# rendeirolab/stainx

Measured on AMD Instinct MI355X. Metric: megapixels/sec Macenko transform, 64x3x512x512 fp32; max-abs vs torch CPU, higher is better.
Workload: dtype f32; 1 GPU; Macenko reference-mode transform, 64x3x512x512 fp32 per GPU (BASELINE configs[1]); tiles_per_gpu=64, height=512, width=512, input_batches_rotated=2, parallelism=tiles sharded over 1 GPU(s), no collective

## Files before the change

stainx_amd/csrc/macenko.hip:

```cpp
#include "common.hpp"

#include <algorithm>
#include <atomic>
#include <type_traits>
#include <cstdlib>

namespace sx {
namespace macenko {

constexpr int kSample = 4096;
constexpr int kMinCap = 8192;
constexpr int kChunk = 16384;
template <typename T> struct PackOf { static constexpr int n = 16 / (int)sizeof(T); };
constexpr int kSlots = 4;
constexpr int kMoments = 20;
constexpr int kPartial = 10;
constexpr int kShortList = 512;
constexpr int kGroupThreads = 1024;
constexpr int kKeys = kSample / kGroupThreads;
constexpr int kPrefetchHist = 8;
constexpr int kPrefetchCand = 8;
static_assert(kKeys * kGroupThreads == kSample && kPrefetchCand * kGroupThreads <= kMinCap, "per-tile stage geometry");

constexpr float kBeta = 0.15f;
// ... 258 lines not shown
        __syncthreads();
    }
};
template <typename F> struct Coded {
    uint8_t v;
    __device__ __forceinline__ operator uint32_t() const { return v; }
};
template <typename T> struct Sem { using type = T; };
template <typename F> struct Sem<Coded<F>> { using type = F; };
template <typename F> __device__ __forceinline__ float code_value(int k) {
    return Elem<F>::load(Elem<F>::store(div255_of_level((float)k)));
}
template <typename F> struct LevelTables<Coded<F>> {
    float od[256], l2[256];
    __device__ __forceinline__ void fill() {
        for (int t = threadIdx.x; t < 256; t += blockDim.x) {
            const float v = code_value<F>(t);
            od[t] = optical_density<F>(v);
            l2[t] = log2_level<F>(v);
        }
        __syncthreads();
    }
};
template <typename F, int kCodeCopies> struct CodeTable {
    static constexpr int copies = kCodeCopies;
    uint2 e[256 * kCodeCopies];
    __device__ __forceinline__ void fill() {
        for (int t = threadIdx.x; t < 256; t += blockDim.x) {
            const float v = code_value<F>(t);
            const uint2 entry = make_uint2(__float_as_uint(v), __float_as_uint(optical_density<F>(v)));
#pragma unroll
            for (int c = 0; c < kCodeCopies; ++c) e[t * kCodeCopies + c] = entry;
        }
        __syncthreads();
    }
};
template <typename T, int V, bool kInter> struct Codable { static constexpr bool value = std::is_same<T, float>::value && V == 4 && !kInter; };

template <typename T> __device__ __forceinline__ float od_of(float v, const LevelTables<T>& tb) {
    if constexpr (sizeof(T) == 1) return tb.od[__float_as_uint(v)]; else return optical_density<T>(v);
}
template <typename T> __device__ __forceinline__ float l2_of(float v, const LevelTables<T>& tb) {
    if constexpr (sizeof(T) == 1) return tb.l2[__float_as_uint(v)]; else return log2_level<T>(v);
}

__device__ __forceinline__ bool od_selected(const float od[3], bool use_all) {
    return use_all || (fminf(od[0], fminf(od[1], od[2])) >= kBeta);
}

__device__ __forceinline__ float diamond_angle(float t1, float t0) {
    const float den = fmaxf(fabsf(t0) + fabsf(t1), 1e-30f);
    const float r = t1 * __builtin_amdgcn_rcpf(den);
    return t0 >= 0.0f ? r : (t1 >= 0.0f ? 2.0f - r : -2.0f - r);
// ... 147 lines not shown
        }
        return out;
    }
};
__device__ __forceinline__ bool in_mask(uint32_t mask_bits, int i) { return ((mask_bits >> i) & 1u) != 0u; }
__device__ __forceinline__ uint32_t* mask_count_words(const Workspace& ws, int64_t item) { return ws.block_hist + (size_t)item * 512; }
__device__ __forceinline__ float sample_out_of_mask() { return __uint_as_float(0x7FC00000u); }
__device__ __forceinline__ bool sample_in_mask(const float od[3]) { return od[0] == od[0]; }

template <typename T> __device__ __forceinline__ float input_level(float held) {
    if constexpr (sizeof(T) == 1) return (float)__float_as_uint(held); else return held * 255.0f;
}

template <int W>
__device__ __forceinline__ void store_codes(const Geometry& g, const Workspace& ws, int64_t tile, int64_t p, const uint32_t (&word)[3][W]) {
    static_assert(W == 1 || W == 2, "four or eight codes per plane");
#pragma unroll
    for (int c = 0; c < 3; ++c) {
        uint8_t* dst = ws.codes + ((size_t)tile * 3 + c) * g.pixels + p;
        if constexpr (W == 1) *reinterpret_cast<uint32_t*>(dst) = word[c][0]; else *reinterpret_cast<uint2*>(dst) = make_uint2(word[c][0], word[c][1]);
    }
}
template <typename T, int V, bool kInter, class Table>
__device__ __forceinline__ void code_quad(const PixelPacks<T, V, kInter>& u, int i0, const LevelTables<T>& tb, const Table& ct, const Geometry& g, const Workspace& ws, int64_t tile, float (&od_quad)[4][3], uint32_t (&word)[3][V / 4]) {
    static_assert((V == 4 || V == 8) && !kInter, "a pack's codes are one or two 32-bit words of a plane");
    constexpr int kCodeCopies = Table::copies;
    uint32_t differ = 0u;
    const int copy = (int)(threadIdx.x % kCodeCopies);
#pragma unroll
    for (int c = 0; c < 3; ++c) {
        uint32_t w = 0u;
#pragma unroll
        for (int ii = 0; ii < 4; ++ii) {
            const float x = u.value(c, i0 + ii);
            const uint32_t k = __float_as_uint(fmaf(x, 255.0f, 8388608.0f)) & 0xFFu;
            const uint2 entry = ct.e[k * kCodeCopies + copy];
            differ |= entry.x ^ __float_as_uint(x);
            od_quad[ii][c] = __uint_as_float(entry.y);
            w |= k << (8 * ii);
        }
        word[c][i0 / 4] = w;
    }
    if (__builtin_expect(__builtin_amdgcn_ballot_w64(differ != 0u) != 0ull, 0)) {
#pragma unroll
        for (int ii = 0; ii < 4; ++ii)
#pragma unroll
            for (int c = 0; c < 3; ++c) {
                float x = u.value(c, i0 + ii);
                asm volatile("" : "+v"(x));
                od_quad[ii][c] = od_of<T>(x, tb);
            }
        if (differ != 0u) put(&ws.code_bad[tile], g.code_epoch);
    }
}


template <typename O, int V, bool kInter>
__device__ __forceinline__ void store_pixels(O* __restrict__ dst, int64_t pixels, int64_t p, const O (&res)[3][V]) {
    if constexpr (kInter) {
        O flat[3][V];
#pragma unroll
        for (int i = 0; i < V; ++i)
#pragma unroll
            for (int c = 0; c < 3; ++c) flat[(3 * i + c) / V][(3 * i + c) % V] = res[c][i];
#pragma unroll
        for (int k = 0; k < 3; ++k) store_pack_stream<O, V>(dst + 3 * p + k * V, flat[k]);
    } else {
#pragma unroll
        for (int c = 0; c < 3; ++c) store_pack_stream<O, V>(dst + c * pixels + p, res[c]);
    }
}

template <typename O, int V>
__device__ __forceinline__ void store_pixels_staged(O* __restrict__ dst, int64_t p, const O (&res)[3][V], uint4* __restrict__ stage) {
    static_assert(sizeof(O) * V == 16, "16-byte packs");
// ... 4338 lines not shown
```

stainx_amd/csrc/macenko_twopass.hpp:

```cpp
#pragma once

namespace sx {
namespace macenko {

constexpr int kPriorSweeps = 4;
constexpr int kPriorUnitsMax = kGroupThreads / 4 * kPriorSweeps;
constexpr int kQueue2 = 512;
constexpr float kSpecSigmasConc = 5.0f, kSpecThresholdScale = 1.0f;
constexpr float kSpecSigmas = 5.0f;
constexpr float kSpecEffFar = 2.0f, kSpecEffNear = 1.0f;
__device__ __forceinline__ float spec_eff(const Geometry& g) { return g.prior_step_q16 >= (8u << 16) ? g.spec_eff_far : g.spec_eff_near; }
constexpr float kSpecKw = 0.10f, kSpecKx = 1.3e-3f;
constexpr float kSpecRot = 0.30f;
constexpr uint32_t kSpecSlow = 1u, kSpecHazard = 2u;
constexpr int kMaxSegments = 256;

constexpr int kRowBelowA = 0, kRowAboveA = 1, kRowBelowB = 2, kRowAboveB = 3, kRowConc = 4, kRowW = 8;
struct alignas(128) PriorRecord {
    float a0[3], a1[3], an[3];
    float rows[16][4];
    float kw, kx;
    float cmax[4];
    int32_t mode;
    int32_t min_first;
    uint32_t open;
};

struct alignas(64) FusedTile {
    uint32_t a_done;
    uint32_t s_done;
    uint32_t ncand[kSlots];
    uint32_t pad[10];
};
constexpr int kXcds = 8;
struct alignas(64) FusedQueue {
    uint32_t ticket;
    uint32_t pad[15];
};
struct FusedSched {
    FusedQueue queue[kXcds];
};
static_assert(sizeof(FusedTile) == kFusedTileBytes && sizeof(FusedSched) <= kFusedSchedBytes, "workspace layout");


typedef unsigned int sx_u4 __attribute__((ext_vector_type(4)));
__device__ __forceinline__ uint32_t ld_agent(const uint32_t* p) { return __hip_atomic_load(p, __ATOMIC_RELAXED, __HIP_MEMORY_SCOPE_AGENT); }
__device__ __forceinline__ int32_t ld_agent(const int32_t* p) { return __hip_atomic_load(p, __ATOMIC_RELAXED, __HIP_MEMORY_SCOPE_AGENT); }
__device__ __forceinline__ float ld_agent(const float* p) { return __uint_as_float(__hip_atomic_load(reinterpret_cast<const uint32_t*>(p), __ATOMIC_RELAXED, __HIP_MEMORY_SCOPE_AGENT)); }
// ... 2 lines not shown
}
__device__ __forceinline__ void st_agent(uint32_t* p, uint32_t v) { __hip_atomic_store(p, v, __ATOMIC_RELAXED, __HIP_MEMORY_SCOPE_AGENT); }
__device__ __forceinline__ void st_agent(float* p, float v) { __hip_atomic_store(reinterpret_cast<uint32_t*>(p), __float_as_uint(v), __ATOMIC_RELAXED, __HIP_MEMORY_SCOPE_AGENT); }
__device__ __forceinline__ void st_agent(double* p, double v) {
    __hip_atomic_store(reinterpret_cast<unsigned long long*>(p), (unsigned long long)__double_as_longlong(v), __ATOMIC_RELAXED, __HIP_MEMORY_SCOPE_AGENT);
}
__device__ __forceinline__ void drain_stores() { asm volatile("s_waitcnt vmcnt(0)" ::: "memory"); }

constexpr int kPriorBins = 2048;
constexpr int kPriorAnglePlane = 4;
constexpr float kOpenExponent = 30.0f;
constexpr float kOpenNear = 16.0f;
struct alignas(16) PriorScratch {
    double red[kGroupThreads / kWave][kPartial];
    double mom[kMoments];
    uint32_t hist[5][kPriorBins];
    uint32_t od16[kPriorSweeps][6][kGroupThreads];
    uint32_t n_kept, n_all, hazard, r_max;
    float frame[9];
    float bdir[4][2];
    float bkey[4], blevel[4];
    uint32_t cmax[4];
    uint32_t open;
};

__device__ __forceinline__ uint32_t prior_pick_bin(const uint32_t* hist, uint32_t rank) {
    constexpr int kPer = kPriorBins / kWave;
    static_assert(kPer <= kWave, "second level: one bin per lane");
    const int lane = (int)lane_id();
    uint32_t mine = 0;
#pragma unroll 8
    for (int i = 0; i < kPer; ++i) mine += hist[kPer * lane + i];
    const uint32_t incl = wave_scan_u32(mine);
    const uint64_t over = __ballot(incl > rank);
    const int owner = over ? (__ffsll((long long)over) - 1) : (kWave - 1);
    const uint32_t r = rank - (uint32_t)__builtin_amdgcn_readlane((int)(incl - mine), owner);
    const uint32_t h = lane < kPer ? hist[kPer * owner + lane] : 0u;
    const uint32_t incl2 = wave_scan_u32(h);
    const uint64_t over2 = __ballot(lane < kPer && incl2 > r);
    const int sub = over2 ? (__ffsll((long long)over2) - 1) : (kPer - 1);
    return (uint32_t)(kPer * owner + sub);
}

__device__ __forceinline__ float wave_total_f32(float x) {
    auto step = [](float v, auto mover) { return v + __uint_as_float(mover(__float_as_uint(v))); };
    x = step(x, [](uint32_t b) { return dpp_move<0x111, 0xF>(0u, b); });
// ... 19 lines not shown
#pragma unroll
        for (int i = 0; i < 4; ++i) {
            float v[3][1];
            load_pixels<T, 1, kInter>(img, g.pixels, p + i, v);
#pragma unroll
            for (int c = 0; c < 3; ++c) u[c][i] = v[c][0];
        }
    }
    return have;
}
template <typename T>
__device__ __forceinline__ void prior_densities(const float (&u)[3][4], float (&od)[4][3]) {
#pragma unroll
    for (int i = 0; i < 4; ++i)
#pragma unroll
        for (int c = 0; c < 3; ++c) od[i][c] = optical_density<T>(u[c][i]);
}

template <typename T, bool kVec, bool kInter>
__global__ __launch_bounds__(kGroupThreads) void prior_kernel(const T* __restrict__ images, Geometry g, Workspace ws) {
    __shared__ PriorScratch sh;
    const int tile = blockIdx.x, tid = threadIdx.x, wave = tid / kWave;
    const uint32_t lane = lane_id();
    GroupState& st = ws.state[tile];
    PriorRecord* pr = &ws.prior[tile];
    const T* img = images + (int64_t)tile * 3 * g.pixels;
    SX_STAMP(st, 0);
    if (tid < kSlots) {
        put(&st.ncand[tid], 0u);
        put(&st.below[tid], 0u);
        put(&st.ncand_seen[tid], 0u);
        put(&st.over_count[tid], 0u);
    }
    if (tid < 2) put(&st.phi_pub[tid], 0ull);
    if ((g.fused || g.dense) && tid < (int)(sizeof(FusedTile) / 4)) put(reinterpret_cast<uint32_t*>(&ws.ftile[tile]) + tid, 0u);
    if (g.fused && tile == 0 && tid >= 32 && tid < 32 + kXcds) put(&ws.fsched->queue[tid - 32].ticket, 0u);
    if (tid == 0) {
        put(&st.fell_back, 0u);
        put(&st.spec, 0u);
        sh.n_kept = sh.n_all = sh.hazard = sh.open = sh.r_max = 0;
        sh.cmax[0] = sh.cmax[1] = sh.cmax[2] = sh.cmax[3] = 0;
    }
    for (int i = tid; i < 5 * kPriorBins; i += kGroupThreads) (&sh.hist[0][0])[i] = 0;

    {
        float m[kPartial];
#pragma unroll
        for (int k = 0; k < kPartial; ++k) m[k] = 0.0f;
        float raw[kPriorSweeps][3][4];
        bool have_quad[kPriorSweeps];
#pragma unroll
        for (int s = 0; s < kPriorSweeps; ++s) have_quad[s] = prior_fetch<T, kVec, kInter>(img, g, s, raw[s]);
#pragma unroll
        for (int s = 0; s < kPriorSweeps; ++s) {
            float od[4][3];
            prior_densities<T>(raw[s], od);
            const bool have = have_quad[s];
#pragma unroll
            for (int q = 0; q < 6; ++q) {
                const int e = 2 * q;
                typedef __fp16 fp16x2 __attribute__((ext_vector_type(2)));
                const fp16x2 h = __builtin_amdgcn_cvt_pkrtz(od[e / 3][e % 3], od[(e + 1) / 3][(e + 1) % 3]);
                sh.od16[s][q][tid] = __builtin_bit_cast(uint32_t, h);
            }
#pragma unroll
            for (int i = 0; i < 4; ++i) {
                const float* o = od[i];
                const float keep = (have && od_selected(o, false)) ? 1.0f : 0.0f;
                const float k0 = keep * o[0], k1 = keep * o[1], k2 = keep * o[2];
                m[0] += keep;
                m[1] += k0;
                m[2] += k1;
                m[3] += k2;
                m[4] = fmaf(k0, o[0], m[4]);
                m[5] = fmaf(k0, o[1], m[5]);
                m[6] = fmaf(k0, o[2], m[6]);
                m[7] = fmaf(k1, o[1], m[7]);
                m[8] = fmaf(k1, o[2], m[8]);
                m[9] = fmaf(k2, o[2], m[9]);
            }
        }
        SX_STAMP(st, 1);
#pragma unroll
        for (int k = 0; k < kPartial; ++k) {
            const float s = wave_total_f32(m[k]);
            if (lane == kWave - 1) sh.red[wave][k] = (double)s;
        }
    }
    __syncthreads();
    if (tid < kMoments) {
        double s = 0.0;
        if (tid < kPartial)
            for (int w = 0; w < kGroupThreads / kWave; ++w) s += sh.red[w][tid];
        sh.mom[tid] = s;
    }
    __syncthreads();
    const int m_kept = (int)sh.mom[0];
    SX_STAMP(st, 2);
    if (tid < 2 && m_kept >= 3) {
        double cov[9];
        float vecs[6];
        bool use_all;
        unsigned long long n_sel;
        plane_from_moments<true>(sh.mom, false, cov, vecs, use_all, n_sel);
        if (tid == 0) {
            const double x0 = vecs[0], y0 = vecs[2], z0 = vecs[4], x1 = vecs[1], y1 = vecs[3], z1 = vecs[5];
            double nx = y0 * z1 - z0 * y1, ny = z0 * x1 - x0 * z1, nz = x0 * y1 - y0 * x1;
            const double n2 = nx * nx + ny * ny + nz * nz;
            const double inv = n2 > 0.0 ? 1.0 / sqrt(n2) : 0.0;
            sh.frame[0] = vecs[0]; sh.frame[1] = vecs[2]; sh.frame[2] = vecs[4];
            sh.frame[3] = vecs[1]; sh.frame[4] = vecs[3]; sh.frame[5] = vecs[5];
            sh.frame[6] = (float)(nx * inv); sh.frame[7] = (float)(ny * inv); sh.frame[8] = (float)(nz * inv);
        }
    }
    __syncthreads();
    auto give_up = [&]() {
        if (tid == 0) {
// ... 261 lines not shown
    for (int s = 0; s < kSlots; ++s) at0[s] = (uint32_t)__builtin_amdgcn_readlane((int)base, s);
    const auto rsrc = __builtin_amdgcn_make_buffer_rsrc(rec_tile, 0, (int)(kSlots * cap * 16u), 0x00020000);
    for (uint32_t i0 = 0; i0 < n; i0 += kWave) {
        const uint32_t i = i0 + lane;
        sx_u4 rec = {0u, 0u, 0u, 0u};
        uint32_t flags = 0;
        if (i < n) {
            rec[0] = queue[0][i];
            rec[1] = queue[1][i];
            rec[2] = queue[2][i];
            flags = queue[3][i];
        }
#pragma unroll
        for (int s = 0; s < kSlots; ++s) {
            const bool has = ((flags >> s) & 1u) != 0;
            const uint64_t mask = __builtin_amdgcn_ballot_w64(has);
            const uint32_t at = at0[s] + rank_in_mask(mask);
            if (has && at < cap) __builtin_amdgcn_raw_buffer_store_b128(rec, rsrc, (int)(((uint32_t)s * cap + at) * 16u), 0, 16);
            at0[s] += (uint32_t)__popcll(mask);
        }
    }
}

template <typename T, int V, int TPB, bool kInter, bool kFused = false, bool kEmit = false>
__device__ __forceinline__ void pass_a_item(const T* __restrict__ images, const Geometry& g, const Workspace& ws, int64_t tile, int chunk_id, int64_t item, PassAScratch<TPB>* sh, const LevelTables<T>& tb,
                                            const CodeTable<T, 2>* __restrict__ ct = nullptr) {
    const int64_t p_begin = (int64_t)chunk_id * g.chunk;
    const int64_t p_end = min(p_begin + (int64_t)g.chunk, g.pixels);
    const T* img = images + tile * 3 * g.pixels;
    GroupState& st = ws.state[tile];
    const PriorRecord* __restrict__ pr = &ws.prior[tile];
    const int wave = __builtin_amdgcn_readfirstlane((int)(threadIdx.x / kWave));
    const bool speculate = get(&pr->mode) == 0;
    typedef _Float16 half8 __attribute__((ext_vector_type(8)));
    typedef float float16v __attribute__((ext_vector_type(16)));
    half8 test_rows;
    {
        const uint32_t l = lane_id(), r = l & 31u, h = l >> 5, row_half = (r >> 2) & 1u, test = (r & 3u) + 4u * (r >> 3);
        const float4 coef = *reinterpret_cast<const float4*>(&pr->rows[test][0]);
        const bool mine = h == row_half;
        test_rows[0] = (_Float16)(mine ? coef.x : 0.0f);
        test_rows[1] = (_Float16)(mine ? coef.y : 0.0f);
        test_rows[2] = (_Float16)(mine ? coef.z : 0.0f);
        test_rows[3] = (_Float16)(mine ? coef.w : 0.0f);
        test_rows[4] = test_rows[5] = test_rows[6] = test_rows[7] = (_Float16)0.0f;
    }
    const float kw = get(&pr->kw), kx = get(&pr->kx);
    if (threadIdx.x < 2) sh->below[threadIdx.x] = 0;

    constexpr int kShortRun = 32 / V > 0 ? 32 / V : 1;
    double acc[kPartial];
#pragma unroll
    for (int k = 0; k < kPartial; ++k) acc[k] = 0.0;
    float m[kPartial];
#pragma unroll
    for (int k = 0; k < kPartial; ++k) m[k] = 0.0f;

    uint32_t (*queue)[kQueue2] = sh->queue[wave];
    uint32_t n_q = 0, have[kSlots] = {0u, 0u, 0u, 0u}, below_a = 0, below_b = 0;
    float* cand_tile = ws.cand_od + (size_t)tile * kSlots * 3 * g.cap2;
    const uint32_t seg = (uint32_t)chunk_id * (TPB / kWave) + (uint32_t)wave, seg_base = seg * g.seg_cap;
    auto flush = [&]() {
        if constexpr (kFused)
            write_records_fused(queue, n_q, ws.cand_rec + (size_t)tile * kSlots * g.fused_cap, g.fused_cap, ws.ftile[tile].ncand);
        else
            write_records(queue, n_q, have, cand_tile, g, seg_base, st.over_count);
        n_q = 0;
    };

    const int64_t mine = (int64_t)threadIdx.x * V;
    PixelPacks<T, V, kInter> next;
    next.clear();
    if (p_begin + mine < p_end) next.load(img, g.pixels, p_begin + mine);
    __syncthreads();

    int in_run = 0;
    auto sweep = [&](auto with_tests) {
        constexpr bool kTests = decltype(with_tests)::value;
        constexpr int G = 1;
        for (int64_t base_p = p_begin; base_p < p_end; base_p += (int64_t)TPB * V) {
            const bool live = base_p + mine < p_end;
            const PixelPacks<T, V, kInter> u = next;
            const int64_t p_next = base_p + (int64_t)TPB * V + mine;
            if (p_next < p_end) next.load(img, g.pixels, p_next);
            uint64_t live_mask = __builtin_amdgcn_ballot_w64(live);
            asm volatile("" : "+s"(live_mask));
            float od_quad[4][3];
            if constexpr (kEmit) {
                static_assert(!kEmit || V == 4, "one quad per pack");
                if (live) {
                    uint32_t word[3][1];
                    code_quad(u, 0, tb, *ct, g, ws, tile, od_quad, word);
                    store_codes<1>(g, ws, tile, base_p + mine, word);
                }
            }
#pragma unroll
            for (int i0 = 0; i0 < V; i0 += G) {
                float od[G][3];
                uint64_t valid[G];
                float16v forms[G];
#pragma unroll
                for (int gi = 0; gi < G; ++gi) {
#pragma unroll
                    for (int c = 0; c < 3; ++c) {
                        if constexpr (kEmit) od[gi][c] = od_quad[(i0 + gi) % 4][c]; else od[gi][c] = od_of<T>(u.value(c, i0 + gi), tb);
                    }
                    const bool sel = od_selected(od[gi], false);
                    valid[gi] = __builtin_amdgcn_ballot_w64(sel) & live_mask;
                    if (__builtin_amdgcn_inverse_ballot_w64(valid[gi])) {
                        const float* o = od[gi];
                        m[0] += 1.0f;
                        m[1] += o[0];
                        m[2] += o[1];
                        m[3] += o[2];
                        m[4] = fmaf(o[0], o[0], m[4]);
// ... 18 lines not shown
                    }
                }
                if constexpr (kTests) {
#pragma unroll
                    for (int gi = 0; gi < G; ++gi) {
                        const float* o = od[gi];
                        const float16v& f = forms[gi];
                        const float mrg = fmaf(kw, fabsf(f[kRowW]), fmaf(kx, fabsf(o[0]) + fabsf(o[1]) + fabsf(o[2]), 1e-6f));
                        const uint64_t lt_a = __builtin_amdgcn_ballot_w64(f[kRowBelowA] < -mrg), gt_a = __builtin_amdgcn_ballot_w64(f[kRowAboveA] > mrg);
                        const uint64_t lt_b = __builtin_amdgcn_ballot_w64(f[kRowBelowB] < -mrg), gt_b = __builtin_amdgcn_ballot_w64(f[kRowAboveB] > mrg);
                        below_a += (uint32_t)__popcll(valid[gi] & lt_a);
                        below_b += (uint32_t)__popcll(valid[gi] & lt_b);
                        const uint64_t c_a = valid[gi] & ~lt_a & ~gt_a, c_b = valid[gi] & ~lt_b & ~gt_b;
                        const uint64_t c_c = live_mask & (__builtin_amdgcn_ballot_w64(f[kRowConc] >= -mrg) | __builtin_amdgcn_ballot_w64(f[kRowConc + 1] >= -mrg));
                        const uint64_t c_d = live_mask & (__builtin_amdgcn_ballot_w64(f[kRowConc + 2] >= -mrg) | __builtin_amdgcn_ballot_w64(f[kRowConc + 3] >= -mrg));
                        const uint64_t any = c_a | c_b | c_c | c_d;
                        if (any) {
                            uint32_t flags = __builtin_amdgcn_inverse_ballot_w64(c_a) ? 1u : 0u;
                            flags |= __builtin_amdgcn_inverse_ballot_w64(c_b) ? 2u : 0u;
                            flags |= __builtin_amdgcn_inverse_ballot_w64(c_c) ? 4u : 0u;
                            flags |= __builtin_amdgcn_inverse_ballot_w64(c_d) ? 8u : 0u;
                            if (__builtin_amdgcn_inverse_ballot_w64(any)) {
                                const uint32_t at = n_q + rank_in_mask(any);
                                queue[0][at] = __float_as_uint(o[0]);
                                queue[1][at] = __float_as_uint(o[1]);
                                queue[2][at] = __float_as_uint(o[2]);
                                queue[3][at] = flags;
                            }
                            n_q += (uint32_t)__popcll(any);
                        }
                        if (__builtin_expect(n_q > (uint32_t)(kQueue2 - kWave), 0)) flush();
                    }
                }
                if constexpr (V > 4) __builtin_amdgcn_sched_barrier(0);
            }
            if (++in_run == kShortRun) {
#pragma unroll
                for (int k = 0; k < kPartial; ++k) {
                    acc[k] += (double)m[k];
                    m[k] = 0.0f;
                }
                in_run = 0;
            }
        }
    };
    if (speculate) sweep(std::true_type{}); else sweep(std::false_type{});
    if (in_run) {
#pragma unroll
        for (int k = 0; k < kPartial; ++k) acc[k] += (double)m[k];
    }

    StatsScratch<TPB>* ss = &sh->stats;
#pragma unroll
    for (int k = 0; k < kPartial; ++k) {
// ... 25 lines not shown
    }
    double kept_total = 0.0;
#pragma unroll
    for (int w = 0; w < TPB / kWave; ++w) kept_total += ss->red[w][0];
    if (__builtin_expect(kept_total < 3.0, 0)) {
        if (!tile_has_three_kept_witnesses<T, TPB, kInter>(img, g.pixels)) {
            stats_item_all_pixels<T, V, TPB, kInter>(img, g.pixels, p_begin, p_end, ws.partial_all + item * kPartial, ss);
            if constexpr (kFused) __builtin_amdgcn_fence(__ATOMIC_RELEASE, "agent");
        }
    }
    if constexpr (kFused) {
        drain_stores();
        __syncthreads();
        if (threadIdx.x == 0) __hip_atomic_fetch_add(&ws.ftile[tile].a_done, 1u, __ATOMIC_RELAXED, __HIP_MEMORY_SCOPE_AGENT);
    }
}

template <typename T, int V, bool kInter = false, bool kDense = false>
__global__ __launch_bounds__(kStreamThreads, (Codable<T, V, kInter>::value ? 4 : 1)) void pass_a_kernel(const T* __restrict__ images, Geometry g, Workspace ws) {
    __shared__ PassAScratch<kStreamThreads> sh;
    __shared__ LevelTables<T> tb;
    tb.fill();
    if constexpr (Codable<T, V, kInter>::value) {
        if (g.code_epoch != 0u) {
            __shared__ CodeTable<T, 2> ct;
            ct.fill();
            pass_a_item<T, V, kStreamThreads, kInter, kDense, true>(images, g, ws, blockIdx.x / g.blocks_per_tile, blockIdx.x % g.blocks_per_tile, blockIdx.x, &sh, tb, &ct);
            return;
        }
    }
    pass_a_item<T, V, kStreamThreads, kInter, kDense>(images, g, ws, blockIdx.x / g.blocks_per_tile, blockIdx.x % g.blocks_per_tile, blockIdx.x, &sh, tb);
}

struct PhiBinSetup {
    float inv[9];
    float dir[2][2];
};
struct alignas(128) SlotScratch {
    TileScratch t;
    uint32_t keys[kLdsKeys];
    float vecs[6], pinv[6], he[6];
    double check[8];
    uint32_t lo, hi, n_list, bin, rank_in_bin, result, range_first, range_last, bin_count;
    int ok, use_all;
    unsigned long long n_sel;
    uint32_t seg_prefix[kMaxSegments + 1], seg_total, seg_overflow, over_n;
    uint32_t dense_n;
    uint32_t own_key;
    int partner_ok;
    uint32_t k_floor, k_ceil, n_under;
// ... 70 lines not shown
#pragma unroll
        for (int u = 0; u < kFlight; ++u) {
            const uint32_t o = off + u * team;
#pragma unroll
            for (int c = 0; c < 3; ++c) od[u][c] = o < cnt ? get(&src[(size_t)c * g.cap2 + o]) : 0.0f;
        }
#pragma unroll
        for (int u = 0; u < kFlight; ++u) {
            const uint32_t o = off + u * team;
            if (o < cnt) fn(first + o, od[u]);
        }
    }
}

template <int kPre>
__device__ __forceinline__ void prefetch_candidates_dense(CandPrefetch<kPre>& pf, __amdgpu_buffer_rsrc_t rsrc) {
#pragma unroll
    for (int u = 0; u < kPre; ++u) {
        const sx_u4 rec = __builtin_amdgcn_raw_buffer_load_b128(rsrc, (int)((threadIdx.x + (uint32_t)u * blockDim.x) * 16u), 0, 0);
#pragma unroll
        for (int c = 0; c < 3; ++c) pf.od[u][c] = __uint_as_float(rec[c]);
    }
}
template <int kPre, class Fn>
__device__ __forceinline__ void for_each_candidate_dense(const CandPrefetch<kPre>& pf, uint32_t n, __amdgpu_buffer_rsrc_t rsrc, Fn fn) {
#pragma unroll
    for (int u = 0; u < kPre; ++u) {
        const uint32_t i = threadIdx.x + (uint32_t)u * blockDim.x;
        if (i < n) fn(i, pf.od[u]);
    }
    constexpr int kFlight = 4;
    for (uint32_t i0 = threadIdx.x + (uint32_t)kPre * blockDim.x; i0 < n; i0 += blockDim.x * kFlight) {
        float od[kFlight][3];
#pragma unroll
        for (int u = 0; u < kFlight; ++u) {
            const sx_u4 rec = __builtin_amdgcn_raw_buffer_load_b128(rsrc, (int)((i0 + (uint32_t)u * blockDim.x) * 16u), 0, 0);
#pragma unroll
            for (int c = 0; c < 3; ++c) od[u][c] = __uint_as_float(rec[c]);
        }
#pragma unroll
        for (int u = 0; u < kFlight; ++u) {
            const uint32_t i = i0 + (uint32_t)u * blockDim.x;
            if (i < n) fn(i, od[u]);
        }
    }
}
__device__ __forceinline__ void dense_count(SlotScratch* sh, const Geometry& g, const Workspace& ws, int tile, int slot) {
    if (threadIdx.x == kWave - 1) {
        const uint32_t n_raw = get(&ws.ftile[tile].ncand[slot]);
        sh->seg_total = n_raw;
        sh->dense_n = min(n_raw, g.fused_cap);
        sh->over_n = 0;
        sh->seg_overflow = n_raw > g.fused_cap ? 1u : 0u;
    }
}

__device__ __forceinline__ uint32_t slot_key(const SlotScratch* sh, const uint32_t* __restrict__ spill, uint32_t i) { return i < (uint32_t)kLdsKeys ? sh->keys[i] : get(&spill[i - kLdsKeys]); }

__device__ __forceinline__ void select_prepare(SlotScratch* sh, bool keep_range = false) {
    if (threadIdx.x == 0) {
        if (!keep_range) {
// ... 258 lines not shown
    const float* row2 = pr->rows[kRowConc + 2 * j + 1];
    frame_coordinates(pr, row1, g1);
    frame_coordinates(pr, row2, g2);
    const float u1x = g1[0], u1y = g1[1], t1 = -row1[3], u2x = g2[0], u2y = g2[1], t2 = -row2[3];
    const float det = u1x * u2y - u1y * u2x;
    const float kw = get(&pr->kw), kx = get(&pr->kx);
    if (!(fabsf(det) > 1e-7f)) return false;
    const float inv = __builtin_amdgcn_rcpf(det);
    const float alpha = (gq[0] * u2y - gq[1] * u2x) * inv, beta = (u1x * gq[1] - u1y * gq[0]) * inv;
    const float l1 = fabsf(p[0]) + fabsf(p[1]) + fabsf(p[2]);
    const float rmax = fmaxf(fmaxf(fabsf(row1[0]), fmaxf(fabsf(row1[1]), fabsf(row1[2]))), fmaxf(fabsf(row2[0]), fmaxf(fabsf(row2[1]), fabsf(row2[2]))));
    const bool good = alpha >= 1e-5f * l1 && beta >= 1e-5f * l1 && rmax <= 1.05f && kx >= 1.2e-3f &&
                      (alpha + beta) * kw >= 1.05f * (alpha * fabsf(g1[2]) + beta * fabsf(g2[2]) + fabsf(gq[2])) && (alpha + beta) * (kx - 1.1e-3f) >= 3e-6f * l1 && t1 < 1e30f && t2 < 1e30f;
    theta_out = (double)alpha * (double)t1 + (double)beta * (double)t2;
    const float span = alpha * fmaxf(get(&pr->cmax[2 * j]) - t1, 0.0f) + beta * fmaxf(get(&pr->cmax[2 * j + 1]) - t2, 0.0f);
    hi_out = (float)theta_out + fmaxf(1.25f * span, 1e-3f * fabsf((float)theta_out) + 1e-6f);
    return good;
}

template <typename T, bool kDense = false>
__global__ __launch_bounds__(kGroupThreads) void estimate_stage_kernel(const T* __restrict__ images, Geometry g, Workspace ws, const float* __restrict__ target_max_conc,
                                                                       uint32_t* __restrict__ key_scratch) {
    __shared__ SlotScratch sh;
    const int tile = blockIdx.x >> 1, j = blockIdx.x & 1, slot = 2 + j;
    uint32_t* keep = key_scratch ? key_scratch + ((size_t)tile * 3 + j) * (size_t)g.pixels * (sizeof(T) >= 4 ? sizeof(T) / 4 : 1) : nullptr;
    GroupState& st = ws.state[tile];
    const PriorRecord* pr = &ws.prior[tile];
    const uint32_t below = get(&st.below[j]), spec = get(&st.spec);
    const int mode = get(&pr->mode);
    const bool stamps = j == 0;
    if (stamps) SX_STAMP(st, 8);
    const float* c0 = ws.cand_od + ((size_t)tile * kSlots + j) * 3 * g.cap2;
    const size_t spill_words = kDense ? (g.fused_cap > (uint32_t)kLdsKeys ? g.fused_cap - kLdsKeys : 0u) : (g.cap2 > (uint32_t)kLdsKeys ? g.cap2 - kLdsKeys : 0u);
    uint32_t* const spill_area = kDense ? ws.dense_spill : ws.key_spill;
    const uint4* rec_tile = ws.cand_rec + (size_t)__builtin_amdgcn_readfirstlane(tile) * kSlots * g.fused_cap;
    const auto rsrc_phi = __builtin_amdgcn_make_buffer_rsrc(const_cast<uint4*>(rec_tile + (size_t)__builtin_amdgcn_readfirstlane(j) * g.fused_cap), 0, (int)(g.fused_cap * 16u), 0x00020000);
    const auto rsrc_conc = __builtin_amdgcn_make_buffer_rsrc(const_cast<uint4*>(rec_tile + (size_t)__builtin_amdgcn_readfirstlane(slot) * g.fused_cap), 0, (int)(g.fused_cap * 16u), 0x00020000);
    float v[6];
    bool use_all;
    unsigned long long rank_other;
    {
        exact_moments(g, ws, tile, &sh);
        if (threadIdx.x >= kGroupThreads - (int)(sizeof(PriorRecord) / 4)) {
            const int w = threadIdx.x - (kGroupThreads - (int)(sizeof(PriorRecord) / 4));
            reinterpret_cast<uint32_t*>(&sh.prior)[w] = get(reinterpret_cast<const uint32_t*>(pr) + w);
        }
        if (threadIdx.x == kWave && mode == 0) phi_bin_setup(pr, j, &sh.phi_bins);
        CandPrefetch<8> pf;
        if constexpr (kDense) prefetch_candidates_dense(pf, rsrc_phi); else prefetch_candidates(pf, g, c0);
        select_prepare(&sh);
        if constexpr (kDense) dense_count(&sh, g, ws, tile, j); else segment_prefix(&sh, g, ws, tile, j);
        exact_plane<T>(g, ws, tile, &sh, [&](const float (&vecs)[6]) {
            if (mode == 0) phi_bin_range(&sh.phi_bins, vecs, sh.lo, sh.hi);
        });
#pragma unroll
        for (int i = 0; i < 6; ++i) v[i] = sh.vecs[i];
        if (stamps) SX_STAMP(st, 9);
        const uint32_t n = kDense ? sh.dense_n : sh.seg_prefix[g.n_seg] + sh.over_n, n_raw = sh.seg_total;
        use_all = sh.use_all != 0;
        const unsigned long long n_sel = sh.n_sel;
        const unsigned long long rank = nearest_rank_index(j ? 99.0 : 1.0, n_sel);
        rank_other = nearest_rank_index(j ? 1.0 : 99.0, n_sel);
        bool ok = mode == 0 && (spec & (kSpecSlow | kSpecHazard)) == 0 && !use_all && !g.spec_fail && sh.seg_overflow == 0 && rank >= below && rank - below < n;
        uint32_t* spill = spill_area + ((size_t)tile * kSlots + j) * spill_words;
        uint32_t answer = 0, why = 1u;
        if (ok) {
            double origin, scale;
            slot_bins(&sh, 0u, 0xFFFFFFFFu, origin, scale);
            uint32_t* hist = sh.t.hist_c[0];
            auto phi_key_of = [&](uint32_t i, const float (&od)[3]) {
                const uint32_t k = angle_key(od, v);
                if (i < (uint32_t)kLdsKeys) sh.keys[i] = k; else put(&spill[i - kLdsKeys], k);
                atomicAdd(&hist[bin_of(k, origin, scale)], 1u);
            };
            if constexpr (kDense) for_each_candidate_dense(pf, n, rsrc_phi, phi_key_of); else for_each_candidate(pf, &sh, g, c0, phi_key_of);
            if (threadIdx.x == kGroupThreads - 1) sh.ok = phi_slot_check(&sh.prior, v, j, sh.check, g.spec_rot) ? 1 : 0;
            __syncthreads();
            if (stamps) SX_STAMP(st, 10);
            ok = sh.ok != 0;
            why = 2u;
        }
        if (ok) {
            answer = select_slot_keys(&sh, spill, n, (uint32_t)(rank - below), true);
            const float a = key_float(answer);
            const double slack = 4e-6;
            if (sh.check[2] == 0.0 && !((double)a >= sh.check[0] + slack)) ok = false;
            if (sh.check[3] == 0.0 && !((double)a <= sh.check[1] - slack)) ok = false;
            why = 3u;
        }
        if (!ok) {
            __syncthreads();
            if (threadIdx.x == 0) {
                atomicOr(&st.fell_back, 1u << j);
                atomicOr(&st.spec, (sh.seg_overflow ? 4u : why) << (8 + 4 * j));
                atomicAdd(&ws.state[0].slow_slots, 1u);
            }
            reset_scratch(&sh.t);
            answer = select_whole_group<T>(images, g, tile, j, rank, v, use_all, &sh.t, keep);
        }
        if (threadIdx.x == 0) {
            put(&st.phi_key[j], answer);
            put(&st.rank[j], rank);
            put(&st.ncand_seen[j], mode == 0 ? n_raw : 0u);
            __hip_atomic_store(&st.phi_pub[j], (1ull << 32) | (unsigned long long)answer, __ATOMIC_RELAXED, __HIP_MEMORY_SCOPE_AGENT);
            sh.own_key = answer;
        }
        if (stamps) SX_STAMP(st, 11);
    }
    if (stamps) SX_STAMP(st, 12);
    const float* c1 = ws.cand_od + ((size_t)tile * kSlots + slot) * 3 * g.cap2;
    CandPrefetch<12> pf;
    if constexpr (kDense) prefetch_candidates_dense(pf, rsrc_conc); else prefetch_candidates(pf, g, c1);
    __syncthreads();
    select_prepare(&sh, true);
    if constexpr (kDense) dense_count(&sh, g, ws, tile, slot); else segment_prefix(&sh, g, ws, tile, slot);
    auto vectors_and_check = [&](uint32_t partner_key) {
        float he[6], pinv[6];
        const uint32_t key0 = j == 0 ? sh.own_key : partner_key, key1 = j == 0 ? partner_key : sh.own_key;
        stain_vectors_and_pinv(v, key0, key1, he, pinv);
#pragma unroll
        for (int i = 0; i < 6; ++i) {
            sh.pinv[i] = pinv[i];
            sh.he[i] = he[i];
        }
        double theta = 0.0;
        float hi = 0.0f;
        const bool good = mode == 0 && conc_slot_check(&sh.prior, pinv, j, theta, hi);
        sh.check[0] = theta;
        sh.ok = good ? 1 : 0;
        const double bound = theta + 4e-6 * fabs(theta) + 1e-7;
        uint32_t kf = float_key((float)bound);
        if ((double)key_float(kf) > bound && kf > 0u) --kf;
        sh.k_floor = good ? kf : 0u;
        sh.k_ceil = good ? max(float_key(hi), kf) : 0xFFFFFFFFu;
        sh.lo = sh.k_floor;
// ... 24 lines not shown
    const unsigned long long n_all = (unsigned long long)g.pixels;
    const unsigned long long k99 = nearest_rank_index(99.0, n_all);
    const uint32_t n = kDense ? sh.dense_n : sh.seg_prefix[g.n_seg] + sh.over_n, n_raw = sh.seg_total;
    if (stamps) SX_STAMP(st, 13);
    const unsigned long long outside = n_all - (unsigned long long)n;
    bool ok = mode == 0 && (spec & (kSpecSlow | kSpecHazard)) == 0 && !g.spec_fail && sh.seg_overflow == 0 && k99 >= outside && n > 0;
    uint32_t why = ok && sh.ok == 0 ? 2u : 1u;
    ok = ok && sh.ok != 0;
    uint32_t* spill = spill_area + ((size_t)tile * kSlots + slot) * spill_words;
    uint32_t answer = 0;
    if (ok) {
        const uint32_t k_floor = sh.k_floor, k_ceil = sh.k_ceil;
        uint32_t under = 0u;
        double origin, scale;
        slot_bins(&sh, k_floor, k_ceil, origin, scale);
        uint32_t* hist = sh.t.hist_c[0];
        auto conc_key_of = [&](uint32_t i, const float (&od)[3]) {
            float ca, cb;
            concentration(od, pinv, ca, cb);
            const uint32_t k = float_key(j ? cb : ca);
            if (i < (uint32_t)kLdsKeys) sh.keys[i] = k; else put(&spill[i - kLdsKeys], k);
            if (k < k_floor) ++under; else atomicAdd(&hist[bin_of(k, origin, scale)], 1u);
        };
        if constexpr (kDense) for_each_candidate_dense(pf, n, rsrc_conc, conc_key_of); else for_each_candidate(pf, &sh, g, c1, conc_key_of);
        under = wave_total_u32(under);
        if (lane_id() == 0 && under) atomicAdd(&sh.n_under, under);
        __syncthreads();
        if (stamps) SX_STAMP(st, 14);
        const unsigned long long rank_in = k99 - outside;
        const uint32_t n_under = sh.n_under;
        why = 3u;
        if (rank_in < n_under) {
            ok = false;
        } else {
            answer = select_slot_keys(&sh, spill, n, (uint32_t)(rank_in - n_under), true, nullptr, k_floor, k_ceil);
            const double a = (double)key_float(answer), theta = sh.check[0];
            if (!(a >= theta + 4e-6 * fabs(theta) + 1e-7)) ok = false;
        }
    }
    if (!ok) {
        __syncthreads();
        if (threadIdx.x == 0) {
            atomicOr(&st.fell_back, 1u << slot);
            atomicOr(&st.spec, (sh.seg_overflow ? 4u : why) << (8 + 4 * slot));
            atomicAdd(&ws.state[0].slow_slots, 1u);
        }
        reset_scratch(&sh.t);
// ... 24 lines not shown
```

Measured before the change: 112,900 megapixels/s.

## Store dense candidate records as packed 8-bit level codes instead of float triples

When the prior pass confirms every pixel of a tile sits exactly on a 1/255 level, pass A writes each candidate as one 32-bit word (three 8-bit channel codes plus flags) instead of a 16-byte record of optical-density floats. The estimate stage then loads 4-byte records and recovers the optical densities through a 256-entry shared-memory table. The goal is to cut candidate write and read traffic by four and enlarge the per-wave queue. In exchange it adds a level check in the prior pass, a coded flag in the prior record, an extra table fill, and a fallback that marks the tile slow if a non-level pixel shows up later.

```diff
diff --git a/stainx_amd/csrc/macenko.hip b/stainx_amd/csrc/macenko.hip
--- a/stainx_amd/csrc/macenko.hip
+++ b/stainx_amd/csrc/macenko.hip
@@ -304,13 +304,18 @@
         __syncthreads();
     }
 };
+template <typename F> __device__ __forceinline__ uint2 code_entry(int k) {
+    const float v = code_value<F>(k);
+    return make_uint2(__float_as_uint(v), __float_as_uint(optical_density<F>(v)));
+}
+__device__ __forceinline__ uint32_t nearest_level(float x) { return __float_as_uint(fmaf(x, 255.0f, 8388608.0f)) & 0xFFu; }
+__device__ __forceinline__ uint32_t level_differs(float x, uint32_t entry_x) { return entry_x ^ __float_as_uint(x); }
 template <typename F, int kCodeCopies> struct CodeTable {
     static constexpr int copies = kCodeCopies;
     uint2 e[256 * kCodeCopies];
     __device__ __forceinline__ void fill() {
         for (int t = threadIdx.x; t < 256; t += blockDim.x) {
-            const float v = code_value<F>(t);
-            const uint2 entry = make_uint2(__float_as_uint(v), __float_as_uint(optical_density<F>(v)));
+            const uint2 entry = code_entry<F>(t);
 #pragma unroll
             for (int c = 0; c < kCodeCopies; ++c) e[t * kCodeCopies + c] = entry;
         }
@@ -504,7 +509,8 @@
     }
 }
 template <typename T, int V, bool kInter, class Table>
-__device__ __forceinline__ void code_quad(const PixelPacks<T, V, kInter>& u, int i0, const LevelTables<T>& tb, const Table& ct, const Geometry& g, const Workspace& ws, int64_t tile, float (&od_quad)[4][3], uint32_t (&word)[3][V / 4]) {
+__device__ __forceinline__ void code_quad(const PixelPacks<T, V, kInter>& u, int i0, const LevelTables<T>& tb, const Table& ct, const Geometry& g, const Workspace& ws, int64_t tile, float (&od_quad)[4][3], uint32_t (&word)[3][V / 4],
+                                          uint32_t* also_mark = nullptr, uint32_t mark_bits = 0u) {
     static_assert((V == 4 || V == 8) && !kInter, "a pack's codes are one or two 32-bit words of a plane");
     constexpr int kCodeCopies = Table::copies;
     uint32_t differ = 0u;
@@ -515,9 +521,9 @@
 #pragma unroll
         for (int ii = 0; ii < 4; ++ii) {
             const float x = u.value(c, i0 + ii);
-            const uint32_t k = __float_as_uint(fmaf(x, 255.0f, 8388608.0f)) & 0xFFu;
+            const uint32_t k = nearest_level(x);
             const uint2 entry = ct.e[k * kCodeCopies + copy];
-            differ |= entry.x ^ __float_as_uint(x);
+            differ |= level_differs(x, entry.x);
             od_quad[ii][c] = __uint_as_float(entry.y);
             w |= k << (8 * ii);
         }
@@ -532,7 +538,10 @@
                 asm volatile("" : "+v"(x));
                 od_quad[ii][c] = od_of<T>(x, tb);
             }
-        if (differ != 0u) put(&ws.code_bad[tile], g.code_epoch);
+        if (differ != 0u) {
+            put(&ws.code_bad[tile], g.code_epoch);
+            if (also_mark) atomicOr(also_mark, mark_bits);
+        }
     }
 }
 
diff --git a/stainx_amd/csrc/macenko_twopass.hpp b/stainx_amd/csrc/macenko_twopass.hpp
--- a/stainx_amd/csrc/macenko_twopass.hpp
+++ b/stainx_amd/csrc/macenko_twopass.hpp
@@ -24,6 +24,7 @@
     int32_t mode;
     int32_t min_first;
     uint32_t open;
+    uint32_t coded;
 };
 
 struct alignas(64) FusedTile {
@@ -72,6 +73,7 @@
     float bkey[4], blevel[4];
     uint32_t cmax[4];
     uint32_t open;
+    uint32_t not_level[kGroupThreads / kWave];
 };
 
 __device__ __forceinline__ uint32_t prior_pick_bin(const uint32_t* hist, uint32_t rank) {
@@ -137,6 +139,7 @@
     __shared__ PriorScratch sh;
     const int tile = blockIdx.x, tid = threadIdx.x, wave = tid / kWave;
     const uint32_t lane = lane_id();
+    constexpr bool kCodes = kVec && Codable<T, 4, kInter>::value;
     GroupState& st = ws.state[tile];
     PriorRecord* pr = &ws.prior[tile];
     const T* img = images + (int64_t)tile * 3 * g.pixels;
@@ -166,11 +169,22 @@
         bool have_quad[kPriorSweeps];
 #pragma unroll
         for (int s = 0; s < kPriorSweeps; ++s) have_quad[s] = prior_fetch<T, kVec, kInter>(img, g, s, raw[s]);
+        uint32_t differ = 0u;
 #pragma unroll
         for (int s = 0; s < kPriorSweeps; ++s) {
             float od[4][3];
             prior_densities<T>(raw[s], od);
             const bool have = have_quad[s];
+            if constexpr (kCodes) {
+                if (g.code_epoch != 0u) {
+                    uint32_t d = 0u;
+#pragma unroll
+                    for (int c = 0; c < 3; ++c)
+#pragma unroll
+                        for (int i = 0; i < 4; ++i) d |= level_differs(raw[s][c][i], __float_as_uint(code_value<T>((int)nearest_level(raw[s][c][i]))));
+                    differ |= have ? d : 0u;
+                }
+            }
 #pragma unroll
             for (int q = 0; q < 6; ++q) {
                 const int e = 2 * q;
@@ -201,6 +215,10 @@
             const float s = wave_total_f32(m[k]);
             if (lane == kWave - 1) sh.red[wave][k] = (double)s;
         }
+        if constexpr (kCodes) {
+            const uint64_t any = __ballot(differ != 0u);
+            if (lane == 0) sh.not_level[wave] = any ? 1u : 0u;
+        }
     }
     __syncthreads();
     if (tid < kMoments) {
@@ -208,6 +226,19 @@
         if (tid < kPartial)
             for (int w = 0; w < kGroupThreads / kWave; ++w) s += sh.red[w][tid];
         sh.mom[tid] = s;
+    }
+    if (tid == kWave) {
+        uint32_t coded = 0u;
+        if constexpr (kCodes) {
+            if (g.code_epoch != 0u) {
+                uint32_t bad = 0u;
+#pragma unroll
+                for (int w = 0; w < kGroupThreads / kWave; ++w) bad |= sh.not_level[w];
+                coded = bad ? 0u : 1u;
+                if (bad) put(&ws.code_bad[tile], g.code_epoch);
+            }
+        }
+        put(&pr->coded, coded);
     }
     __syncthreads();
     const int m_kept = (int)sh.mom[0];
@@ -515,7 +546,40 @@
     }
 }
 
-template <typename T, int V, int TPB, bool kInter, bool kFused = false, bool kEmit = false>
+constexpr int kQueueCodes = 4 * kQueue2;
+constexpr int kCodeRecordAux = 16;
+__device__ __forceinline__ void write_records_codes(const uint32_t* __restrict__ queue, uint32_t n, uint4* __restrict__ rec_tile, uint32_t cap, uint32_t* __restrict__ ncand) {
+    if (n == 0) return;
+    const uint32_t lane = lane_id();
+    uint32_t count[kSlots] = {0u, 0u, 0u, 0u};
+    for (uint32_t i0 = 0; i0 < n; i0 += kWave) {
+        const uint32_t i = i0 + lane, flags = i < n ? queue[i] >> 24 : 0u;
+#pragma unroll
+        for (int s = 0; s < kSlots; ++s) count[s] += (uint32_t)__popcll(__builtin_amdgcn_ballot_w64(((flags >> s) & 1u) != 0));
+    }
+    uint32_t base = 0;
+    {
+        const uint32_t mine = lane == 0 ? count[0] : (lane == 1 ? count[1] : (lane == 2 ? count[2] : count[3]));
+        if (lane < (uint32_t)kSlots && mine) base = __hip_atomic_fetch_add(&ncand[lane], mine, __ATOMIC_RELAXED, __HIP_MEMORY_SCOPE_AGENT);
+    }
+    uint32_t at0[kSlots];
+#pragma unroll
+    for (int s = 0; s < kSlots; ++s) at0[s] = (uint32_t)__builtin_amdgcn_readlane((int)base, s);
+    const auto rsrc = __builtin_amdgcn_make_buffer_rsrc(rec_tile, 0, (int)(kSlots * cap * 16u), 0x00020000);
+    for (uint32_t i0 = 0; i0 < n; i0 += kWave) {
+        const uint32_t i = i0 + lane, rec = i < n ? queue[i] : 0u;
+#pragma unroll
+        for (int s = 0; s < kSlots; ++s) {
+            const bool has = ((rec >> (24 + s)) & 1u) != 0;
+            const uint64_t mask = __builtin_amdgcn_ballot_w64(has);
+            const uint32_t at = at0[s] + rank_in_mask(mask);
+            if (has && at < cap) __builtin_amdgcn_raw_buffer_store_b32(rec, rsrc, (int)((uint32_t)s * cap * 16u + at * 4u), 0, kCodeRecordAux);
+            at0[s] += (uint32_t)__popcll(mask);
+        }
+    }
+}
+
+template <typename T, int V, int TPB, bool kInter, bool kFused = false, bool kEmit = false, bool kCodeRec = false>
 __device__ __forceinline__ void pass_a_item(const T* __restrict__ images, const Geometry& g, const Workspace& ws, int64_t tile, int chunk_id, int64_t item, PassAScratch<TPB>* sh, const LevelTables<T>& tb,
                                             const CodeTable<T, 2>* __restrict__ ct = nullptr) {
     const int64_t p_begin = (int64_t)chunk_id * g.chunk;
@@ -549,12 +613,17 @@
 #pragma unroll
     for (int k = 0; k < kPartial; ++k) m[k] = 0.0f;
 
+    static_assert(!kCodeRec || (kFused && kEmit), "code records: dense arrays, looked-up optical densities");
     uint32_t (*queue)[kQueue2] = sh->queue[wave];
+    uint32_t* const queue_codes = &sh->queue[wave][0][0];
+    constexpr uint32_t kQueueRoom = kCodeRec ? kQueueCodes : kQueue2;
     uint32_t n_q = 0, have[kSlots] = {0u, 0u, 0u, 0u}, below_a = 0, below_b = 0;
     float* cand_tile = ws.cand_od + (size_t)tile * kSlots * 3 * g.cap2;
     const uint32_t seg = (uint32_t)chunk_id * (TPB / kWave) + (uint32_t)wave, seg_base = seg * g.seg_cap;
     auto flush = [&]() {
-        if constexpr (kFused)
+        if constexpr (kCodeRec)
+            write_records_codes(queue_codes, n_q, ws.cand_rec + (size_t)tile * kSlots * g.fused_cap, g.fused_cap, ws.ftile[tile].ncand);
+        else if constexpr (kFused)
             write_records_fused(queue, n_q, ws.cand_rec + (size_t)tile * kSlots * g.fused_cap, g.fused_cap, ws.ftile[tile].ncand);
         else
             write_records(queue, n_q, have, cand_tile, g, seg_base, st.over_count);
@@ -579,11 +648,11 @@
             uint64_t live_mask = __builtin_amdgcn_ballot_w64(live);
             asm volatile("" : "+s"(live_mask));
             float od_quad[4][3];
+            uint32_t word[3][1] = {{0u}, {0u}, {0u}};
             if constexpr (kEmit) {
                 static_assert(!kEmit || V == 4, "one quad per pack");
                 if (live) {
-                    uint32_t word[3][1];
-                    code_quad(u, 0, tb, *ct, g, ws, tile, od_quad, word);
+                    if constexpr (kCodeRec) code_quad(u, 0, tb, *ct, g, ws, tile, od_quad, word, &st.spec, kSpecSlow); else code_quad(u, 0, tb, *ct, g, ws, tile, od_quad, word);
                     store_codes<1>(g, ws, tile, base_p + mine, word);
                 }
             }
@@ -648,14 +717,19 @@
                             flags |= __builtin_amdgcn_inverse_ballot_w64(c_d) ? 8u : 0u;
                             if (__builtin_amdgcn_inverse_ballot_w64(any)) {
                                 const uint32_t at = n_q + rank_in_mask(any);
-                                queue[0][at] = __float_as_uint(o[0]);
-                                queue[1][at] = __float_as_uint(o[1]);
-                                queue[2][at] = __float_as_uint(o[2]);
-                                queue[3][at] = flags;
+                                if constexpr (kCodeRec) {
+                                    const int at_byte = 8 * ((i0 + gi) % 4);
+                                    queue_codes[at] = ((word[0][0] >> at_byte) & 0xFFu) | (((word[1][0] >> at_byte) & 0xFFu) << 8) | (((word[2][0] >> at_byte) & 0xFFu) << 16) | (flags << 24);
+                                } else {
+                                    queue[0][at] = __float_as_uint(o[0]);
+                                    queue[1][at] = __float_as_uint(o[1]);
+                                    queue[2][at] = __float_as_uint(o[2]);
+                                    queue[3][at] = flags;
+                                }
                             }
                             n_q += (uint32_t)__popcll(any);
                         }
-                        if (__builtin_expect(n_q > (uint32_t)(kQueue2 - kWave), 0)) flush();
+                        if (__builtin_expect(n_q > kQueueRoom - (uint32_t)kWave, 0)) flush();
                     }
                 }
                 if constexpr (V > 4) __builtin_amdgcn_sched_barrier(0);
@@ -727,10 +801,10 @@
     __shared__ LevelTables<T> tb;
     tb.fill();
     if constexpr (Codable<T, V, kInter>::value) {
-        if (g.code_epoch != 0u) {
+        if (g.code_epoch != 0u && (!kDense || get(&ws.prior[blockIdx.x / g.blocks_per_tile].coded) != 0u)) {
             __shared__ CodeTable<T, 2> ct;
             ct.fill();
-            pass_a_item<T, V, kStreamThreads, kInter, kDense, true>(images, g, ws, blockIdx.x / g.blocks_per_tile, blockIdx.x % g.blocks_per_tile, blockIdx.x, &sh, tb, &ct);
+            pass_a_item<T, V, kStreamThreads, kInter, kDense, true, kDense>(images, g, ws, blockIdx.x / g.blocks_per_tile, blockIdx.x % g.blocks_per_tile, blockIdx.x, &sh, tb, &ct);
             return;
         }
     }
@@ -847,21 +921,50 @@
         for (int c = 0; c < 3; ++c) pf.od[u][c] = __uint_as_float(rec[c]);
     }
 }
+template <int kPre> struct CodePrefetch {
+    uint32_t rec[kPre];
+};
+template <int kPre>
+__device__ __forceinline__ void prefetch_candidates_codes(CodePrefetch<kPre>& pc, __amdgpu_buffer_rsrc_t rsrc) {
+#pragma unroll
+    for (int u = 0; u < kPre; ++u) pc.rec[u] = __builtin_amdgcn_raw_buffer_load_b32(rsrc, (int)((threadIdx.x + (uint32_t)u * blockDim.x) * 4u), 0, 0);
+}
+__device__ __forceinline__ void code_record_densities(uint32_t rec, const float* __restrict__ od_of_code, float (&od)[3]) {
+#pragma unroll
+    for (int c = 0; c < 3; ++c) od[c] = od_of_code[(rec >> (8 * c)) & 0xFFu];
+}
 template <int kPre, class Fn>
-__device__ __forceinline__ void for_each_candidate_dense(const CandPrefetch<kPre>& pf, uint32_t n, __amdgpu_buffer_rsrc_t rsrc, Fn fn) {
+__device__ __forceinline__ void for_each_candidate_dense(const CandPrefetch<kPre>& pf, const CodePrefetch<kPre>& pc, bool codes, const float* __restrict__ od_of_code, uint32_t n, __amdgpu_buffer_rsrc_t rsrc, Fn fn) {
 #pragma unroll
     for (int u = 0; u < kPre; ++u) {
         const uint32_t i = threadIdx.x + (uint32_t)u * blockDim.x;
-        if (i < n) fn(i, pf.od[u]);
+        if (i < n) {
+            float od[3];
+            if (codes) {
+                code_record_densities(pc.rec[u], od_of_code, od);
+            } else {
+#pragma unroll
+                for (int c = 0; c < 3; ++c) od[c] = pf.od[u][c];
+            }
+            fn(i, od);
+        }
     }
     constexpr int kFlight = 4;
     for (uint32_t i0 = threadIdx.x + (uint32_t)kPre * blockDim.x; i0 < n; i0 += blockDim.x * kFlight) {
         float od[kFlight][3];
-#pragma unroll
-        for (int u = 0; u < kFlight; ++u) {
-            const sx_u4 rec = __builtin_amdgcn_raw_buffer_load_b128(rsrc, (int)((i0 + (uint32_t)u * blockDim.x) * 16u), 0, 0);
-#pragma unroll
-            for (int c = 0; c < 3; ++c) od[u][c] = __uint_as_float(rec[c]);
+        if (codes) {
+            uint32_t rec[kFlight];
+#pragma unroll
+            for (int u = 0; u < kFlight; ++u) rec[u] = __builtin_amdgcn_raw_buffer_load_b32(rsrc, (int)((i0 + (uint32_t)u * blockDim.x) * 4u), 0, 0);
+#pragma unroll
+            for (int u = 0; u < kFlight; ++u) code_record_densities(rec[u], od_of_code, od[u]);
+        } else {
+#pragma unroll
+            for (int u = 0; u < kFlight; ++u) {
+                const sx_u4 rec = __builtin_amdgcn_raw_buffer_load_b128(rsrc, (int)((i0 + (uint32_t)u * blockDim.x) * 16u), 0, 0);
+#pragma unroll
+                for (int c = 0; c < 3; ++c) od[u][c] = __uint_as_float(rec[c]);
+            }
         }
 #pragma unroll
         for (int u = 0; u < kFlight; ++u) {
@@ -1166,12 +1269,16 @@
 __global__ __launch_bounds__(kGroupThreads) void estimate_stage_kernel(const T* __restrict__ images, Geometry g, Workspace ws, const float* __restrict__ target_max_conc,
                                                                        uint32_t* __restrict__ key_scratch) {
     __shared__ SlotScratch sh;
+    constexpr bool kCodeRec = kDense && Codable<T, 4, false>::value;
+    __shared__ float od_of_code[kCodeRec ? 256 : 1];
     const int tile = blockIdx.x >> 1, j = blockIdx.x & 1, slot = 2 + j;
     uint32_t* keep = key_scratch ? key_scratch + ((size_t)tile * 3 + j) * (size_t)g.pixels * (sizeof(T) >= 4 ? sizeof(T) / 4 : 1) : nullptr;
     GroupState& st = ws.state[tile];
     const PriorRecord* pr = &ws.prior[tile];
     const uint32_t below = get(&st.below[j]), spec = get(&st.spec);
     const int mode = get(&pr->mode);
+    bool coded = false;
+    if constexpr (kCodeRec) coded = g.code_epoch != 0u && get(&pr->coded) != 0u;
     const bool stamps = j == 0;
     if (stamps) SX_STAMP(st, 8);
     const float* c0 = ws.cand_od + ((size_t)tile * kSlots + j) * 3 * g.cap2;
@@ -1191,7 +1298,15 @@
         }
         if (threadIdx.x == kWave && mode == 0) phi_bin_setup(pr, j, &sh.phi_bins);
         CandPrefetch<8> pf;
-        if constexpr (kDense) prefetch_candidates_dense(pf, rsrc_phi); else prefetch_candidates(pf, g, c0);
+        CodePrefetch<8> pc;
+        if constexpr (kDense) {
+            if (coded) prefetch_candidates_codes(pc, rsrc_phi); else prefetch_candidates_dense(pf, rsrc_phi);
+        } else {
+            prefetch_candidates(pf, g, c0);
+        }
+        if constexpr (kCodeRec) {
+            if (coded && threadIdx.x < 256) od_of_code[threadIdx.x] = __uint_as_float(code_entry<T>((int)threadIdx.x).y);
+        }
         select_prepare(&sh);
         if constexpr (kDense) dense_count(&sh, g, ws, tile, j); else segment_prefix(&sh, g, ws, tile, j);
         exact_plane<T>(g, ws, tile, &sh, [&](const float (&vecs)[6]) {
@@ -1217,7 +1332,7 @@
                 if (i < (uint32_t)kLdsKeys) sh.keys[i] = k; else put(&spill[i - kLdsKeys], k);
                 atomicAdd(&hist[bin_of(k, origin, scale)], 1u);
             };
-            if constexpr (kDense) for_each_candidate_dense(pf, n, rsrc_phi, phi_key_of); else for_each_candidate(pf, &sh, g, c0, phi_key_of);
+            if constexpr (kDense) for_each_candidate_dense(pf, pc, coded, od_of_code, n, rsrc_phi, phi_key_of); else for_each_candidate(pf, &sh, g, c0, phi_key_of);
             if (threadIdx.x == kGroupThreads - 1) sh.ok = phi_slot_check(&sh.prior, v, j, sh.check, g.spec_rot) ? 1 : 0;
             __syncthreads();
             if (stamps) SX_STAMP(st, 10);
@@ -1254,7 +1369,12 @@
     if (stamps) SX_STAMP(st, 12);
     const float* c1 = ws.cand_od + ((size_t)tile * kSlots + slot) * 3 * g.cap2;
     CandPrefetch<12> pf;
-    if constexpr (kDense) prefetch_candidates_dense(pf, rsrc_conc); else prefetch_candidates(pf, g, c1);
+    CodePrefetch<12> pc;
+    if constexpr (kDense) {
+        if (coded) prefetch_candidates_codes(pc, rsrc_conc); else prefetch_candidates_dense(pf, rsrc_conc);
+    } else {
+        prefetch_candidates(pf, g, c1);
+    }
     __syncthreads();
     select_prepare(&sh, true);
     if constexpr (kDense) dense_count(&sh, g, ws, tile, slot); else segment_prefix(&sh, g, ws, tile, slot);
@@ -1325,7 +1445,7 @@
             if (i < (uint32_t)kLdsKeys) sh.keys[i] = k; else put(&spill[i - kLdsKeys], k);
             if (k < k_floor) ++under; else atomicAdd(&hist[bin_of(k, origin, scale)], 1u);
         };
-        if constexpr (kDense) for_each_candidate_dense(pf, n, rsrc_conc, conc_key_of); else for_each_candidate(pf, &sh, g, c1, conc_key_of);
+        if constexpr (kDense) for_each_candidate_dense(pf, pc, coded, od_of_code, n, rsrc_conc, conc_key_of); else for_each_candidate(pf, &sh, g, c1, conc_key_of);
         under = wave_total_u32(under);
         if (lane_id() == 0 && under) atomicAdd(&sh.n_under, under);
         __syncthreads();
```

Result: faster. 115,900 megapixels/s, median of 6 (+2.7%).
